# Project-MONAI/GenerativeModels

Measured on NVIDIA H100. Metric: ddim50_voxels_per_s, higher is better.
Workload: dtype fp16

## Files before the change

### generativemodels_b200/csrc/igemm.cu

```cuda
#include "common.cuh"
#include "wgmma.cuh"
#include <cuda.h>
#include <cudaTypedefs.h>
#include <mutex>
#include <string.h>

namespace b200 {

static constexpr int kBM = 128;
static constexpr int kBK = 64;
static constexpr int kABytes = kBM * kBK * 2;
static constexpr int kMmaWarp0 = 4;
static constexpr int kTmaWarp = 12;
static constexpr int kThreads = 13 * 32;

struct SegDev {
  int8_t src, dw, dh, dd;
  uint16_t c0, nchunks;
};

struct IgemmDev {
  alignas(64) CUtensorMap tmA[2];
  alignas(64) CUtensorMap tmB;
  const h16* a_ptr[2];
  int a_C[2], a_pitch[2];
  int in_N, in_D, in_H, in_W;
  int a_bcast;
  const h16* w_ptr;
  int w_rows, w_K, w_pitch;
  long long w_bstride;
  int w_batched;
  int n_seg, num_k_chunks;
  int sd, sh, sw;
  int N, OD, OH, OW;
  int BW, BH, BD, bw_log2, bh_log2;
  int tiles_w, tiles_h, tiles_d, tiles_n, num_tiles;
  int k_splits;
  long long split_stride;
  void* out_ptr;
  int out_dtype, cout, out_cols, out_vec, out_staged, out_v256;
  float* stat_ptr;
  float* gn_partial;
  int gn_slots, gn_slot0;
  int gn_sh;
  long long out_sN, out_sD, out_sH, out_sW;
  const float* bias;
  const float* rowvec;
  long long rowvec_bstride;
  const float* row_bias;
  int act1, act2;
  int geglu;
  float scale;
  const void* res_ptr;
  int res_dtype, res_vec, res_v256;
  long long res_sN, res_sD, res_sH, res_sW;
  SegDev seg[B200_IGEMM_MAX_SEG];
};

__device__ __forceinline__ void tma_load_5d(const CUtensorMap* tm, uint32_t bar, uint32_t dst, int c0,
                                            int c1, int c2, int c3, int c4) {
  asm volatile(
      "cp.async.bulk.tensor.5d.shared::cluster.global.mbarrier::complete_tx::bytes"
      " [%0], [%1, {%3, %4, %5, %6, %7}], [%2];" ::"r"(dst),
      "l"(reinterpret_cast<uint64_t>(tm)), "r"(bar), "r"(c0), "r"(c1), "r"(c2), "r"(c3), "r"(c4)
      : "memory");
}
template <int CH>
__device__ __forceinline__ void acc_ld(const float* src, uint32_t* r) {
#pragma unroll
  for (int j = 0; j < CH; j += 4) {
    const float4 t = *reinterpret_cast<const float4*>(src + j);
    r[j] = __float_as_uint(t.x); r[j + 1] = __float_as_uint(t.y);
    r[j + 2] = __float_as_uint(t.z); r[j + 3] = __float_as_uint(t.w);
  }
}

__host__ __device__ __forceinline__ int split_begin(int num_k, int splits, int ks) {
  return (int)(((long long)num_k * ks) / splits);
}

template <int CH>
__device__ __forceinline__ void epilogue_math(const IgemmDev& p, float* v, int nb, int ow, long long res_off,
                                              int col0) {
  const float rb = p.row_bias ? __ldg(p.row_bias + ow) : 0.f;
#pragma unroll
  for (int j = 0; j < CH; ++j) {
    int col = col0 + j;
    float add = rb;
    if (col < p.cout) {
      if (p.bias) add += __ldg(p.bias + col);
      if (p.rowvec) add += __ldg(p.rowvec + (long long)nb * p.rowvec_bstride + col);
    }
    float x = v[j] + add;
    x = apply_act(x, p.act1);
    v[j] = x * p.scale;
  }
  if (p.res_ptr) {
    if (p.res_dtype == B200_DT_H16) {
      const h16* r = reinterpret_cast<const h16*>(p.res_ptr) + res_off + col0;
      if (p.res_vec) {
#pragma unroll
        for (int g = 0; g < CH / 8; ++g) {
          if (col0 + g * 8 < p.out_cols) {
            uint4 t = __ldg(reinterpret_cast<const uint4*>(r + g * 8));
            float f[8];
            unpack8(t, f);
#pragma unroll
            for (int j = 0; j < 8; ++j) v[g * 8 + j] += f[j];
          }
        }
      } else {
#pragma unroll
        for (int j = 0; j < CH; ++j)
          if (col0 + j < p.out_cols) v[j] += h2f(r[j]);
      }
    } else {
      const float* r = reinterpret_cast<const float*>(p.res_ptr) + res_off + col0;
      if (p.res_vec) {
#pragma unroll
        for (int g = 0; g < CH / 4; ++g) {
          if (col0 + g * 4 < p.out_cols) {
            float4 t = __ldg(reinterpret_cast<const float4*>(r + g * 4));
            v[g * 4 + 0] += t.x; v[g * 4 + 1] += t.y; v[g * 4 + 2] += t.z; v[g * 4 + 3] += t.w;
          }
        }
      } else {
#pragma unroll
        for (int j = 0; j < CH; ++j)
          if (col0 + j < p.out_cols) v[j] += r[j];
      }
    }
  }
  if (p.act2 != B200_ACT_NONE) {
#pragma unroll
    for (int j = 0; j < CH; ++j) v[j] = apply_act(v[j], p.act2);
  }
#pragma unroll
  for (int j = 0; j < CH; ++j)
    if (col0 + j >= p.cout) v[j] = 0.f;
}

template <int CH>
__device__ __forceinline__ void store_direct(const IgemmDev& p, const float* v, long long out_off, int col0) {
  if (p.out_dtype == B200_DT_H16) {
    h16* o = reinterpret_cast<h16*>(p.out_ptr) + out_off + col0;
    if (p.out_vec) {
#pragma unroll
      for (int g = 0; g < CH / 8; ++g)
        if (col0 + g * 8 < p.out_cols) *reinterpret_cast<uint4*>(o + g * 8) = pack8(v + g * 8);
    } else {
#pragma unroll
      for (int j = 0; j < CH; ++j)
        if (col0 + j < p.out_cols) o[j] = f2h(v[j]);
    }
  } else {
    float* o = reinterpret_cast<float*>(p.out_ptr) + out_off + col0;
    if (p.out_vec) {
#pragma unroll
      for (int g = 0; g < CH / 4; ++g)
        if (col0 + g * 4 < p.out_cols)
          *reinterpret_cast<float4*>(o + g * 4) =
              make_float4(v[g * 4], v[g * 4 + 1], v[g * 4 + 2], v[g * 4 + 3]);
    } else {
#pragma unroll
      for (int j = 0; j < CH; ++j)
        if (col0 + j < p.out_cols) o[j] = v[j];
    }
  }
}


__device__ __forceinline__ void ldg256(const void* ptr, uint4& a, uint4& b) {
  a = __ldg(reinterpret_cast<const uint4*>(ptr));
  b = __ldg(reinterpret_cast<const uint4*>(ptr) + 1);
}
__device__ __forceinline__ void stg256(void* ptr, const uint4& a, const uint4& b) {
  reinterpret_cast<uint4*>(ptr)[0] = a;
  reinterpret_cast<uint4*>(ptr)[1] = b;
}
template <int CH>
__device__ __forceinline__ void act_inplace(float* v, int act) {
  if (act == B200_ACT_NONE) return;
  if (act == B200_ACT_SILU) {
#pragma unroll
    for (int j = 0; j < CH; ++j) v[j] = silu_f(v[j]);
  } else if (act == B200_ACT_LEAKYRELU || act == B200_ACT_LEAKYRELU02) {
    const float slope = act == B200_ACT_LEAKYRELU ? 0.01f : 0.2f;
#pragma unroll
    for (int j = 0; j < CH; ++j) v[j] = v[j] > 0.0f ? v[j] : slope * v[j];
  } else if (act == B200_ACT_GELU) {
#pragma unroll
    for (int j = 0; j < CH; ++j) v[j] = 0.5f * v[j] * (1.0f + erff(v[j] * 0.70710678118654752f));
  } else if (act == B200_ACT_TANH || act == B200_ACT_SIGMOID) {
#pragma unroll
    for (int j = 0; j < CH; ++j) v[j] = apply_act(v[j], act);
  } else {
#pragma unroll
    for (int j = 0; j < CH; ++j) v[j] = fmaxf(v[j], 0.0f);
  }
}
template <int CH>
__device__ __forceinline__ void load_res_fast(const IgemmDev& p, uint4* rv, long long res_off, int col0) {
  const h16* r = reinterpret_cast<const h16*>(p.res_ptr) + res_off + col0;
  if (p.res_v256) {
#pragma unroll
    for (int g = 0; g < CH / 16; ++g) ldg256(r + g * 16, rv[2 * g], rv[2 * g + 1]);
  } else {
#pragma unroll
    for (int g = 0; g < CH / 8; ++g) rv[g] = __ldg(reinterpret_cast<const uint4*>(r + g * 8));
  }
}
template <int CH>
__device__ __forceinline__ void epilogue_fast(const IgemmDev& p, const uint32_t* raw, const float* addv,
                                              const uint4* rv, long long out_off, int col0, float* gs) {
  float v[CH];
#pragma unroll
  for (int j = 0; j < CH; j += 4) {
    const float4 a = *reinterpret_cast<const float4*>(addv + j);
    v[j] = __uint_as_float(raw[j]) + a.x;
// ... 368 lines not shown
              h16* o = reinterpret_cast<h16*>(p.out_ptr) + out_off + ((n0 + c0) >> 1);
              uint4 pk[4];
#pragma unroll
              for (int g = 0; g < 4; ++g) pk[g] = pack8(v + g * 8);
              if (p.out_v256) {
                stg256(o, pk[0], pk[1]);
                stg256(o + 16, pk[2], pk[3]);
              } else {
#pragma unroll
                for (int g = 0; g < 4; ++g) *reinterpret_cast<uint4*>(o + g * 8) = pk[g];
              }
            }
          }
          c0 = BN;
        }
      }
      if (lean_ok) {
#pragma unroll 1
        for (; c0 < BN && n0 + c0 + CH <= p.cout; c0 += CH) {
          uint4 rv[CH / 8];
#pragma unroll
          for (int g = 0; g < CH / 8; ++g) rv[g] = rv_next[g];
          if (res_fast && c0 + CH < BN && n0 + c0 + 2 * CH <= p.cout)
            load_res_fast<CH>(p, rv_next, res_off, n0 + c0 + CH);
          uint32_t raw[CH];
          acc_ld<CH>(acc_row + c0, raw);
          if (row_ok) {
            if (p.res_ptr) epilogue_lean<CH, true>(p, raw, addv + c0, rv, out_off, n0 + c0);
            else epilogue_lean<CH, false>(p, raw, addv + c0, rv, out_off, n0 + c0);
          }
        }
      }
#pragma unroll 1
      for (; c0 < BN; c0 += CH) {
        if (n0 + c0 >= p.out_cols) break;
        if (fast_ok && n0 + c0 + CH <= p.cout) {
          uint4 rv[CH / 8];
#pragma unroll
          for (int g = 0; g < CH / 8; ++g) rv[g] = rv_next[g];
          if (res_fast && c0 + CH < BN && n0 + c0 + 2 * CH <= p.cout)
            load_res_fast<CH>(p, rv_next, res_off, n0 + c0 + CH);
          uint32_t raw[CH];
          acc_ld<CH>(acc_row + c0, raw);
          float gs[16] = {0.f, 0.f, 0.f, 0.f, 0.f, 0.f, 0.f, 0.f, 0.f, 0.f, 0.f, 0.f, 0.f, 0.f, 0.f, 0.f};
          if (row_ok) {
            if (p.row_bias) {
              const float rb = __ldg(p.row_bias + ow);
#pragma unroll
              for (int j = 0; j < CH; ++j) raw[j] = __float_as_uint(__uint_as_float(raw[j]) + rb);
            }
            epilogue_fast<CH>(p, raw, addv + c0, rv, out_off, n0 + c0, gn_on ? gs : nullptr);
          }
          if constexpr (CH == 32) {
            if (gn_on && p.gn_sh == 2) {
              float a8[8], a4[4], a2[2];
              bool hi = (lane & 16) != 0;
#pragma unroll
              for (int i = 0; i < 8; ++i) {
                const float send = hi ? gs[i] : gs[8 + i], keep = hi ? gs[8 + i] : gs[i];
                a8[i] = keep + __shfl_xor_sync(0xffffffffu, send, 16);
              }
              hi = (lane & 8) != 0;
#pragma unroll
              for (int i = 0; i < 4; ++i) {
                const float send = hi ? a8[i] : a8[4 + i], keep = hi ? a8[4 + i] : a8[i];
                a4[i] = keep + __shfl_xor_sync(0xffffffffu, send, 8);
              }
              hi = (lane & 4) != 0;
#pragma unroll
              for (int i = 0; i < 2; ++i) {
                const float send = hi ? a4[i] : a4[2 + i], keep = hi ? a4[2 + i] : a4[i];
                a2[i] = keep + __shfl_xor_sync(0xffffffffu, send, 4);
              }
              hi = (lane & 2) != 0;
              float c = (hi ? a2[1] : a2[0]) + __shfl_xor_sync(0xffffffffu, hi ? a2[0] : a2[1], 2);
              c += __shfl_xor_sync(0xffffffffu, c, 1);
              if ((lane & 1) == 0) {
                const int grp = (c0 >> 2) + ((lane >> 3) & 1) * 4 + ((lane >> 2) & 1) * 2 + ((lane >> 1) & 1);
                gacc[grp * 2 + (lane >> 4)] += c;
              }
            } else if (gn_on) {
              float a[4], b[2];
              bool hi = (lane & 16) != 0;
#pragma unroll
              for (int i = 0; i < 4; ++i) {
                const float send = hi ? gs[i] : gs[4 + i], keep = hi ? gs[4 + i] : gs[i];
                a[i] = keep + __shfl_xor_sync(0xffffffffu, send, 16);
              }
              hi = (lane & 8) != 0;
#pragma unroll
              for (int i = 0; i < 2; ++i) {
                const float send = hi ? a[i] : a[2 + i], keep = hi ? a[2 + i] : a[i];
                b[i] = keep + __shfl_xor_sync(0xffffffffu, send, 8);
              }
              hi = (lane & 4) != 0;
              float c = (hi ? b[1] : b[0]) + __shfl_xor_sync(0xffffffffu, hi ? b[0] : b[1], 4);
              c += __shfl_xor_sync(0xffffffffu, c, 2);
              c += __shfl_xor_sync(0xffffffffu, c, 1);
              if ((lane & 3) == 0) {
                const int grp = (c0 >> 3) + ((lane >> 3) & 1) * 2 + ((lane >> 2) & 1);
                gacc[grp * 2 + (lane >> 4)] += c;
              }
            }
          }
          continue;
        }
        uint32_t raw[CH];
        acc_ld<CH>(acc_row + c0, raw);
        float v[CH];
#pragma unroll
        for (int j = 0; j < CH; ++j) v[j] = __uint_as_float(raw[j]);
        if (row_ok) epilogue_math<CH>(p, v, nb, ow, res_off, n0 + c0);
        if (p.stat_ptr && row_ok) {
          float cmax = -INFINITY;
#pragma unroll
          for (int j = 0; j < CH; ++j)
            if (n0 + c0 + j < p.cout) cmax = fmaxf(cmax, v[j]);
          if (cmax > -INFINITY) {
            const float nm = fmaxf(run_max, cmax);
            float acc = 0.f;
#pragma unroll
            for (int j = 0; j < CH; ++j)
              if (n0 + c0 + j < p.cout) acc += __expf(v[j] - nm);
            run_sum = run_sum * __expf(run_max - nm) + acc;
            run_max = nm;
          }
        }
        if (p.out_staged) store_staged<CH>(p, v, my_tile, row_ok, out_off, n0 + c0, lane);
        else if (row_ok) store_direct<CH>(p, v, out_off, n0 + c0);
      }
      if (p.stat_ptr && row_ok) {
        float2* st = reinterpret_cast<float2*>(p.stat_ptr) + ((long long)ow * p.tiles_n + nt);
        *st = make_float2(run_max, run_sum);
      }
      if (want_key >= 0) {
#pragma unroll
        for (int i = 0; i < PER; ++i)
          if (lane + 32 * i < BN) addv_other[lane + 32 * i] = nbv[i] + nrw[i];
        next_key = want_key;
      }
      __syncwarp();
      if (lane == 0) mbar_arrive(tempty_bar);
    }
    if (gn_on) { __syncwarp(); gn_flush(); }
  }

  __syncthreads();
}

namespace wide {
static constexpr int kThreads = 384;
static constexpr int kCluster = 2;
static constexpr int kBN = 256;
static constexpr int kStages = 4;
static constexpr int kBHalfBytes = 128 * kBK * 2;
static constexpr int kStageBytes = kABytes + 2 * kBHalfBytes;
static constexpr int kSliceLd = 36;
static constexpr int kOffSlice = kStages * kStageBytes;
static constexpr int kOffAdd = kOffSlice + 8 * 16 * kSliceLd * 4;
static constexpr int kOffBar = kOffAdd + 8 * kBN * 4;
static constexpr int kSmem = 1024 + kOffBar + 2 * kStages * 8;
static constexpr int kProducerRegs = 40, kConsumerRegs = 232;
static_assert(kProducerRegs * 128 + kConsumerRegs * 256 <= 65536, "register budget of one CTA per SM");
}

__device__ __forceinline__ float gn_reduce16(const float* gs, int lane, int gn_sh) {
  const bool h3 = (lane & 8) != 0, h2 = (lane & 4) != 0, h1 = (lane & 2) != 0;
  if (gn_sh == 3) {
    float a[2];
#pragma unroll
    for (int i = 0; i < 2; ++i) a[i] = (h3 ? gs[2 + i] : gs[i]) + __shfl_xor_sync(0xffffffffu, h3 ? gs[i] : gs[2 + i], 8);
    float c = (h2 ? a[1] : a[0]) + __shfl_xor_sync(0xffffffffu, h2 ? a[0] : a[1], 4);
    c += __shfl_xor_sync(0xffffffffu, c, 2);
    c += __shfl_xor_sync(0xffffffffu, c, 1);
    return c;
  }
  float a4[4], a2[2];
#pragma unroll
  for (int i = 0; i < 4; ++i) a4[i] = (h3 ? gs[4 + i] : gs[i]) + __shfl_xor_sync(0xffffffffu, h3 ? gs[i] : gs[4 + i], 8);
#pragma unroll
  for (int i = 0; i < 2; ++i) a2[i] = (h2 ? a4[2 + i] : a4[i]) + __shfl_xor_sync(0xffffffffu, h2 ? a4[i] : a4[2 + i], 4);
  float c = (h1 ? a2[1] : a2[0]) + __shfl_xor_sync(0xffffffffu, h1 ? a2[0] : a2[1], 2);
  c += __shfl_xor_sync(0xffffffffu, c, 1);
  return c;
}

__global__ void __launch_bounds__(wide::kThreads, 1) igemm_wide_kernel(const __grid_constant__ IgemmDev p) {
  using namespace wide;
  extern __shared__ uint8_t smem_raw[];
  uint8_t* sm = smem_raw + ((1024u - (smem_u32(smem_raw) & 1023u)) & 1023u);
  const uint32_t ring = smem_u32(sm);
  const uint32_t full0 = ring + kOffBar, empty0 = full0 + 8 * kStages;

  const int tid = threadIdx.x;
  const int wg = __shfl_sync(0xffffffffu, tid >> 7, 0);
  const uint32_t rank = cluster_ctarank();
  const int cid = (int)blockIdx.x / kCluster, n_clusters = (int)gridDim.x / kCluster;
  const int m_tiles = p.tiles_w * p.tiles_h * p.tiles_d * p.N;
  const int num_units = p.num_tiles;
  const int num_k = p.num_k_chunks;

  if (tid == 0) {
    for (int s = 0; s < kStages; ++s) {
      mbar_init(full0 + 8 * s, 1);
      mbar_init(empty0 + 8 * s, 8 * kCluster);
    }
    asm volatile("fence.mbarrier_init.release.cluster;" ::: "memory");
  }
  cluster_sync();

  struct MTile { int nt, wt, ht, dt, nb; bool ok; };
  auto unit_tile = [&](int u) {
    MTile t;
    t.nt = u % p.tiles_n;
    int m = 2 * (u / p.tiles_n) + (int)rank;
    t.ok = m < m_tiles;
    if (!t.ok) m = m_tiles - 1;
    t.wt = m % p.tiles_w; m /= p.tiles_w;
    t.ht = m % p.tiles_h; m /= p.tiles_h;
    t.dt = m % p.tiles_d;
    t.nb = m / p.tiles_d;
    return t;
  };

  if (wg == 0) {
    setmaxnreg_dec<kProducerRegs>();
    if (tid == 0) {
      int stage = 0;
      uint32_t phase = 0;
      for (int u = cid; u < num_units; u += n_clusters) {
        const MTile t = unit_tile(u);
        const int iw0 = t.wt * p.BW * p.sw, ih0 = t.ht * p.BH * p.sh, id0 = t.dt * p.BD * p.sd;
        const int wrow = t.nt * kBN + 128 * (int)rank;
        int kglob = 0;
        for (int s = 0; s < p.n_seg; ++s) {
          const SegDev sg = p.seg[s];
          const CUtensorMap* tm = &p.tmA[sg.src];
          const int cw = iw0 + sg.dw, ch = ih0 + sg.dh, cd = id0 + sg.dd;
          for (int c = 0; c < sg.nchunks; ++c, ++kglob) {
            mbar_wait(empty0 + 8 * stage, phase ^ 1u);
            const uint32_t dst = ring + stage * kStageBytes, fb = full0 + 8 * stage;
            mbar_arrive_expect_tx(fb, kStageBytes);
            tma_load_5d(tm, fb, dst, (sg.c0 + c) * kBK, cw, ch, cd, t.nb);
            tma_load_3d_multicast(&p.tmB, fb, dst + kABytes + rank * kBHalfBytes, kglob * kBK, wrow, 0, 0x3);
            if (++stage == kStages) { stage = 0; phase ^= 1u; }
          }
        }
      }
    }
  } else {
    setmaxnreg_inc<kConsumerRegs>();
    const int c = wg - 1;
    const int wq = (tid >> 5) & 3;
    const int lane = tid & 31;
    float* slice = reinterpret_cast<float*>(sm + kOffSlice) + (4 * c + wq) * 16 * kSliceLd;
    float* addv = reinterpret_cast<float*>(sm + kOffAdd) + (4 * c + wq) * kBN;
    const int er = 64 * c + 16 * wq + (lane & 15);
    const int eh = lane >> 4;
    const int rw = er & (p.BW - 1), rh = (er >> p.bw_log2) & (p.BH - 1), rd = er >> (p.bw_log2 + p.bh_log2);
    auto release = [&](int s) {
      __syncwarp();
      if (lane == 0) {
        mbar_arrive_cluster(empty0 + 8 * s, 0);
        mbar_arrive_cluster(empty0 + 8 * s, 1);
      }
    };

    const bool gn_on = p.gn_partial != nullptr;
    const int gsh = p.gn_sh;
    float gacc[kBN / 32];
#pragma unroll
    for (int s = 0; s < kBN / 32; ++s) gacc[s] = 0.f;
    int key = -1, gn_nb = 0, gn_n0 = 0;
    auto gn_flush = [&]() {
      const bool writer = (lane & (gsh == 3 ? 3 : 1)) == 0;
      const int stat = (lane >> 3) & 1;
      const int gl = gsh == 3 ? (lane >> 2) & 1 : ((lane >> 1) & 3);
      float* dst = p.gn_partial +
                   (((long long)gn_nb * p.gn_slots + p.gn_slot0 + 4 * blockIdx.x + wq) * (p.cout >> gsh)) * 2 + stat;
      for (int pass = 0; pass < 2; ++pass) {
        if (pass == c && writer) {
#pragma unroll
          for (int s = 0; s < kBN / 32; ++s) dst[(((gn_n0 + 32 * s + 16 * eh) >> gsh) + gl) * 2] += gacc[s];
        }
        if (pass == 0) named_sync(1, 256);
      }
#pragma unroll
      for (int s = 0; s < kBN / 32; ++s) gacc[s] = 0.f;
    };

    float acc[kBN / 2];
    int stage = 0;
    uint32_t phase = 0;
    for (int u = cid; u < num_units; u += n_clusters) {
      int prev = -1;
      for (int k = 0; k < num_k; ++k) {
        mbar_wait(full0 + 8 * stage, phase);
        const uint32_t st = ring + stage * kStageBytes;
        const uint64_t adesc = wgmma_desc(st + c * (64 * kBK * 2));
        const uint64_t bdesc = wgmma_desc(st + kABytes);
        wgmma_fence();
#pragma unroll
        for (int kk = 0; kk < kBK / 16; ++kk)
          wgmma_ss<kBN>(acc, adesc + 2u * kk, bdesc + 2u * kk, (k | kk) != 0 ? 1u : 0u);
        wgmma_commit();
        wgmma_wait<1>();
        if (prev >= 0) release(prev);
        prev = stage;
        if (++stage == kStages) { stage = 0; phase ^= 1u; }
      }
      wgmma_wait<0>();
      wgmma_touch<kBN / 2>(acc);
      release(prev);

      const MTile t = unit_tile(u);
      const int n0 = t.nt * kBN;
      const int ow = t.wt * p.BW + rw, oh = t.ht * p.BH + rh, od = t.dt * p.BD + rd;
      const bool row_ok = t.ok && ow < p.OW && oh < p.OH && od < p.OD;
      const long long out_off = t.nb * p.out_sN + od * p.out_sD + oh * p.out_sH + ow * p.out_sW;
      const long long res_off = t.nb * p.res_sN + od * p.res_sD + oh * p.res_sH + ow * p.res_sW;
      if (t.nb * p.tiles_n + t.nt != key) {
        if (gn_on && key >= 0) gn_flush();
        key = t.nb * p.tiles_n + t.nt;
        gn_nb = t.nb;
        gn_n0 = n0;
        float bv[kBN / 32], rv[kBN / 32];
#pragma unroll
        for (int i = 0; i < kBN / 32; ++i) {
          const int col = n0 + lane + 32 * i;
          bv[i] = p.bias ? __ldg(p.bias + col) : 0.f;
          rv[i] = p.rowvec ? __ldg(p.rowvec + (long long)t.nb * p.rowvec_bstride + col) : 0.f;
        }
        __syncwarp();
#pragma unroll
        for (int i = 0; i < kBN / 32; ++i) addv[lane + 32 * i] = bv[i] + rv[i];
        __syncwarp();
      }
      const bool res_on = p.res_ptr && row_ok;
      uint4 rv_next[2] = {make_uint4(0u, 0u, 0u, 0u), make_uint4(0u, 0u, 0u, 0u)};
      if (res_on) load_res_fast<16>(p, rv_next, res_off, n0 + 16 * eh);
#pragma unroll
      for (int s = 0; s < kBN / 32; ++s) {
        __syncwarp();
#pragma unroll
        for (int j = 4 * s; j < 4 * s + 4; ++j) {
          const int col = 8 * (j - 4 * s) + 2 * (lane & 3);
          *reinterpret_cast<float2*>(slice + (lane >> 2) * kSliceLd + col) = make_float2(acc[4 * j], acc[4 * j + 1]);
          *reinterpret_cast<float2*>(slice + ((lane >> 2) + 8) * kSliceLd + col) =
              make_float2(acc[4 * j + 2], acc[4 * j + 3]);
        }
        __syncwarp();
        uint32_t raw[16];
        acc_ld<16>(slice + (lane & 15) * kSliceLd + 16 * eh, raw);
        const uint4 rv[2] = {rv_next[0], rv_next[1]};
        if (res_on && s + 1 < kBN / 32) load_res_fast<16>(p, rv_next, res_off, n0 + 32 * (s + 1) + 16 * eh);
        const int cc = 32 * s + 16 * eh;
        float gs[8] = {0.f, 0.f, 0.f, 0.f, 0.f, 0.f, 0.f, 0.f};
        if (row_ok) epilogue_fast<16>(p, raw, addv + cc, rv, out_off, n0 + cc, gs);
        if (gn_on) gacc[s] += gn_reduce16(gs, lane, gsh);
      }
    }
    if (gn_on && key >= 0) gn_flush();
  }
  cluster_sync();
}

__global__ void igemm_check_kernel(const __grid_constant__ IgemmDev p) {
  const long long rows = (long long)p.N * p.OD * p.OH * p.OW;
  const int col_groups = (p.out_cols + 15) / 16;
  const long long idx = (long long)blockIdx.x * blockDim.x + threadIdx.x;
  if (idx >= rows * col_groups) return;
  const int cg = (int)(idx % col_groups);
  long long m = idx / col_groups;
  const int ow = (int)(m % p.OW); m /= p.OW;
  const int oh = (int)(m % p.OH); m /= p.OH;
  const int od = (int)(m % p.OD); m /= p.OD;
  const int nb = (int)m;
  float acc[16];
#pragma unroll
  for (int j = 0; j < 16; ++j) acc[j] = 0.f;
  const int wb = p.w_batched ? nb : 0;
  const h16* wbase = p.w_ptr + (long long)wb * p.w_bstride;
  int kglob = 0;
  for (int s = 0; s < p.n_seg; ++s) {
    const SegDev sg = p.seg[s];
    const int iw = ow * p.sw + sg.dw, ih = oh * p.sh + sg.dh, id = od * p.sd + sg.dd;
    const bool inb = iw >= 0 && iw < p.in_W && ih >= 0 && ih < p.in_H && id >= 0 && id < p.in_D;
    const h16* a = p.a_ptr[sg.src] +
        ((((long long)(p.a_bcast ? 0 : nb) * p.in_D + id) * p.in_H + ih) * p.in_W + iw) * p.a_pitch[sg.src];
    for (int c = 0; c < sg.nchunks; ++c, ++kglob) {
      if (!inb) continue;
      for (int e = 0; e < kBK; ++e) {
        const int ch = (sg.c0 + c) * kBK + e;
        const int kk = kglob * kBK + e;
        if (ch >= p.a_C[sg.src] || kk >= p.w_K) break;
        const float av = h2f(a[ch]);
#pragma unroll
        for (int j = 0; j < 16; ++j) {
          const int col = cg * 16 + j;
          if (col < p.w_rows) acc[j] += av * h2f(wbase[(long long)col * p.w_pitch + kk]);
        }
      }
    }
  }
  const long long out_off = nb * p.out_sN + od * p.out_sD + oh * p.out_sH + ow * p.out_sW;
  const long long res_off = nb * p.res_sN + od * p.res_sD + oh * p.res_sH + ow * p.res_sW;
  epilogue_row<16>(p, acc, nb, ow, out_off, res_off, cg * 16);
}

static PFN_cuTensorMapEncodeTiled g_encode = nullptr;
static std::once_flag g_encode_once;

static void load_encode() {
  void* fn = nullptr;
  cudaDriverEntryPointQueryResult qres;
  if (cudaGetDriverEntryPoint("cuTensorMapEncodeTiled", &fn, cudaEnableDefault, &qres) == cudaSuccess &&
      qres == cudaDriverEntryPointSuccess)
    g_encode = reinterpret_cast<PFN_cuTensorMapEncodeTiled>(fn);
}

static int ilog2(int v) {
  int l = 0;
  while ((1 << l) < v) ++l;
  return l;
}

struct TileShape { int bw, bh, bd; };

static TileShape choose_tile(int OW, int OH, int OD, int sw, int sh, int sd) {
  static const TileShape cands[] = {{128, 1, 1}, {64, 2, 1}, {32, 4, 1}, {16, 8, 1}, {8, 16, 1},
                                    {4, 32, 1},  {32, 2, 2}, {16, 4, 2}, {8, 8, 2},  {16, 2, 4},
                                    {8, 4, 4},   {4, 8, 4},  {4, 4, 8},  {8, 2, 8},  {2, 8, 8},
                                    {4, 2, 16},  {2, 4, 16}, {2, 2, 32}, {1, 1, 128}, {1, 128, 1},
                                    {2, 64, 1},  {1, 8, 16}, {1, 16, 8}};
  double best = 1e30;
  TileShape bt = cands[0];
  for (const TileShape& c : cands) {
    if (c.bw * sw > 256 || c.bh * sh > 256 || c.bd * sd > 256) continue;
    double tw = (double)((OW + c.bw - 1) / c.bw) * c.bw;
    double th = (double)((OH + c.bh - 1) / c.bh) * c.bh;
    double td = (double)((OD + c.bd - 1) / c.bd) * c.bd;
    double cost = tw * th * td;
    cost *= (1.0 + 1e-3 * (7 - ilog2(c.bw)));
    if (cost < best) { best = cost; bt = c; }
  }
  return bt;
}

__global__ void gn8_partial_check_kernel(const __grid_constant__ IgemmDev p) {
  const long long rows = (long long)p.N * p.OD * p.OH * p.OW;
  const int gw = 1 << p.gn_sh;
  const int groups = p.cout >> p.gn_sh;
  const long long idx = (long long)blockIdx.x * blockDim.x + threadIdx.x;
  if (idx >= rows * groups) return;
  const int g = (int)(idx % groups);
  long long m = idx / groups;
  const int ow = (int)(m % p.OW); m /= p.OW;
  const int oh = (int)(m % p.OH); m /= p.OH;
  const int od = (int)(m % p.OD); m /= p.OD;
  const int nb = (int)m;
  const h16* o = reinterpret_cast<const h16*>(p.out_ptr) + nb * p.out_sN + od * p.out_sD +
                           oh * p.out_sH + ow * p.out_sW + g * gw;
  float s = 0.f, q = 0.f;
  for (int j = 0; j < gw; ++j) { const float f = h2f(o[j]); s += f; q = fmaf(f, f, q); }
  float* dst = p.gn_partial + (((long long)nb * p.gn_slots + p.gn_slot0) * groups + g) * 2;
  atomicAdd(dst, s);
  atomicAdd(dst + 1, q);
}

__global__ void __launch_bounds__(256) igemm_split_reduce_kernel(const IgemmDev p, const float* __restrict__ ws,
                                                                 int splits, int ws_cols, long long ws_stride) {
  const int groups = (p.out_cols + 7) >> 3;
  const long long rows = (long long)p.N * p.OD * p.OH * p.OW;
  const long long idx = blockIdx.x * (long long)blockDim.x + threadIdx.x;
  if (idx >= rows * groups) return;
  const int col0 = (int)(idx % groups) * 8;
  const long long row = idx / groups;
  long long t = row;
  const int ow = (int)(t % p.OW); t /= p.OW;
  const int oh = (int)(t % p.OH); t /= p.OH;
  const int od = (int)(t % p.OD); t /= p.OD;
  const int nb = (int)t;
  float v[8] = {0.f, 0.f, 0.f, 0.f, 0.f, 0.f, 0.f, 0.f};
  const float* src = ws + row * ws_cols + col0;
  int s = 0;
  for (; s + 8 <= splits; s += 8, src += 8 * ws_stride) {
    float4 a[8], b[8];
#pragma unroll
    for (int j = 0; j < 8; ++j) {
      a[j] = __ldg(reinterpret_cast<const float4*>(src + j * ws_stride));
      b[j] = __ldg(reinterpret_cast<const float4*>(src + j * ws_stride + 4));
    }
#pragma unroll
    for (int j = 0; j < 8; ++j) {
      v[0] += a[j].x; v[1] += a[j].y; v[2] += a[j].z; v[3] += a[j].w;
      v[4] += b[j].x; v[5] += b[j].y; v[6] += b[j].z; v[7] += b[j].w;
    }
  }
  if (s + 4 <= splits) {
    float4 a[4], b[4];
#pragma unroll
    for (int j = 0; j < 4; ++j) {
      a[j] = __ldg(reinterpret_cast<const float4*>(src + j * ws_stride));
      b[j] = __ldg(reinterpret_cast<const float4*>(src + j * ws_stride + 4));
    }
#pragma unroll
    for (int j = 0; j < 4; ++j) {
      v[0] += a[j].x; v[1] += a[j].y; v[2] += a[j].z; v[3] += a[j].w;
      v[4] += b[j].x; v[5] += b[j].y; v[6] += b[j].z; v[7] += b[j].w;
    }
    s += 4; src += 4 * ws_stride;
  }
  if (s + 2 <= splits) {
    const float4 a0 = __ldg(reinterpret_cast<const float4*>(src)), b0 = __ldg(reinterpret_cast<const float4*>(src + 4));
    const float4 a1 = __ldg(reinterpret_cast<const float4*>(src + ws_stride));
// ... 367 lines not shown
```

Measured before the change: 145,500.

## Stage wide-kernel epilogue through shared memory with bulk residual loads and row stores

```diff
diff --git a/generativemodels_b200/csrc/igemm.cu b/generativemodels_b200/csrc/igemm.cu
--- a/generativemodels_b200/csrc/igemm.cu
+++ b/generativemodels_b200/csrc/igemm.cu
@@ -65,6 +65,14 @@
       "l"(reinterpret_cast<uint64_t>(tm)), "r"(bar), "r"(c0), "r"(c1), "r"(c2), "r"(c3), "r"(c4)
       : "memory");
 }
+__device__ __forceinline__ void bulk_load(uint32_t dst, const void* src, uint32_t bytes, uint32_t bar) {
+  asm volatile("cp.async.bulk.shared::cluster.global.mbarrier::complete_tx::bytes [%0], [%1], %2, [%3];"
+               ::"r"(dst), "l"(src), "r"(bytes), "r"(bar) : "memory");
+}
+__device__ __forceinline__ void bulk_store(void* dst, uint32_t src, uint32_t bytes) {
+  asm volatile("cp.async.bulk.global.shared::cta.bulk_group [%0], [%1], %2;" ::"l"(dst), "r"(src), "r"(bytes)
+               : "memory");
+}
 template <int CH>
 __device__ __forceinline__ void acc_ld(const float* src, uint32_t* r) {
 #pragma unroll
@@ -739,35 +747,30 @@
 static constexpr int kThreads = 384;
 static constexpr int kCluster = 2;
 static constexpr int kBN = 256;
-static constexpr int kStages = 4;
+static constexpr int kStages = 3;
 static constexpr int kBHalfBytes = 128 * kBK * 2;
 static constexpr int kStageBytes = kABytes + 2 * kBHalfBytes;
-static constexpr int kSliceLd = 36;
-static constexpr int kOffSlice = kStages * kStageBytes;
-static constexpr int kOffAdd = kOffSlice + 8 * 16 * kSliceLd * 4;
+static constexpr int kRowBytes = kBN * 2;
+static constexpr int kStgLd = kRowBytes + 16;
+static constexpr int kOffStg = kStages * kStageBytes;
+static constexpr int kOffAdd = kOffStg + kBM * kStgLd;
 static constexpr int kOffBar = kOffAdd + 8 * kBN * 4;
-static constexpr int kSmem = 1024 + kOffBar + 2 * kStages * 8;
+static constexpr int kSmem = 1024 + kOffBar + (2 * kStages + 2) * 8;
 static constexpr int kProducerRegs = 40, kConsumerRegs = 232;
 static_assert(kProducerRegs * 128 + kConsumerRegs * 256 <= 65536, "register budget of one CTA per SM");
 }
 
-__device__ __forceinline__ float gn_reduce16(const float* gs, int lane, int gn_sh) {
-  const bool h3 = (lane & 8) != 0, h2 = (lane & 4) != 0, h1 = (lane & 2) != 0;
-  if (gn_sh == 3) {
-    float a[2];
-#pragma unroll
-    for (int i = 0; i < 2; ++i) a[i] = (h3 ? gs[2 + i] : gs[i]) + __shfl_xor_sync(0xffffffffu, h3 ? gs[i] : gs[2 + i], 8);
-    float c = (h2 ? a[1] : a[0]) + __shfl_xor_sync(0xffffffffu, h2 ? a[0] : a[1], 4);
-    c += __shfl_xor_sync(0xffffffffu, c, 2);
-    c += __shfl_xor_sync(0xffffffffu, c, 1);
-    return c;
-  }
-  float a4[4], a2[2];
-#pragma unroll
-  for (int i = 0; i < 4; ++i) a4[i] = (h3 ? gs[4 + i] : gs[i]) + __shfl_xor_sync(0xffffffffu, h3 ? gs[i] : gs[4 + i], 8);
-#pragma unroll
-  for (int i = 0; i < 2; ++i) a2[i] = (h2 ? a4[2 + i] : a4[i]) + __shfl_xor_sync(0xffffffffu, h2 ? a4[i] : a4[2 + i], 4);
-  float c = (h1 ? a2[1] : a2[0]) + __shfl_xor_sync(0xffffffffu, h1 ? a2[0] : a2[1], 2);
+__device__ __forceinline__ float gn_reduce_slice(const float* s, int lane, int gn_sh) {
+  float a[4], b[2];
+  bool hi = (lane & 16) != 0;
+#pragma unroll
+  for (int i = 0; i < 4; ++i) a[i] = (hi ? s[4 + i] : s[i]) + __shfl_xor_sync(0xffffffffu, hi ? s[i] : s[4 + i], 16);
+  hi = (lane & 8) != 0;
+#pragma unroll
+  for (int i = 0; i < 2; ++i) b[i] = (hi ? a[2 + i] : a[i]) + __shfl_xor_sync(0xffffffffu, hi ? a[i] : a[2 + i], 8);
+  hi = (lane & 4) != 0;
+  float c = (hi ? b[1] : b[0]) + __shfl_xor_sync(0xffffffffu, hi ? b[0] : b[1], 4);
+  if (gn_sh == 3) c += __shfl_xor_sync(0xffffffffu, c, 2);
   c += __shfl_xor_sync(0xffffffffu, c, 1);
   return c;
 }
@@ -778,6 +781,7 @@
   uint8_t* sm = smem_raw + ((1024u - (smem_u32(smem_raw) & 1023u)) & 1023u);
   const uint32_t ring = smem_u32(sm);
   const uint32_t full0 = ring + kOffBar, empty0 = full0 + 8 * kStages;
+  const uint32_t stg = ring + kOffStg, stg_full = empty0 + 8 * kStages, stg_empty = stg_full + 8;
 
   const int tid = threadIdx.x;
   const int wg = __shfl_sync(0xffffffffu, tid >> 7, 0);
@@ -792,6 +796,8 @@
       mbar_init(full0 + 8 * s, 1);
       mbar_init(empty0 + 8 * s, 8 * kCluster);
     }
+    mbar_init(stg_full, 1);
+    mbar_init(stg_empty, 8);
     asm volatile("fence.mbarrier_init.release.cluster;" ::: "memory");
   }
   cluster_sync();
@@ -809,9 +815,16 @@
     t.nb = m / p.tiles_d;
     return t;
   };
+  auto tile_row = [&](const MTile& t, int r, int& ow, int& oh, int& od) {
+    ow = t.wt * p.BW + (r & (p.BW - 1));
+    oh = t.ht * p.BH + ((r >> p.bw_log2) & (p.BH - 1));
+    od = t.dt * p.BD + (r >> (p.bw_log2 + p.bh_log2));
+    return t.ok && ow < p.OW && oh < p.OH && od < p.OD;
+  };
 
   if (wg == 0) {
     setmaxnreg_dec<kProducerRegs>();
+    const int warp = __shfl_sync(0xffffffffu, tid >> 5, 0);
     if (tid == 0) {
       int stage = 0;
       uint32_t phase = 0;
@@ -834,17 +847,36 @@
           }
         }
       }
+    } else if (warp == 1 && p.res_ptr) {
+      const int lane = tid & 31;
+      uint32_t it = 0;
+      for (int u = cid; u < num_units; u += n_clusters, ++it) {
+        const MTile t = unit_tile(u);
+        mbar_wait(stg_empty, (it & 1u) ^ 1u);
+        int ow, oh, od, rows = 0;
+#pragma unroll
+        for (int i = 0; i < kBM / 32; ++i) rows += __popc(__ballot_sync(0xffffffffu, tile_row(t, lane + 32 * i, ow, oh, od)));
+        if (lane == 0) mbar_arrive_expect_tx(stg_full, rows * kRowBytes);
+        __syncwarp();
+#pragma unroll
+        for (int i = 0; i < kBM / 32; ++i) {
+          const int r = lane + 32 * i;
+          if (tile_row(t, r, ow, oh, od)) {
+            const h16* src = reinterpret_cast<const h16*>(p.res_ptr) + t.nb * p.res_sN + od * p.res_sD +
+                             oh * p.res_sH + ow * p.res_sW + t.nt * kBN;
+            bulk_load(stg + r * kStgLd, src, kRowBytes, stg_full);
+          }
+        }
+      }
     }
   } else {
     setmaxnreg_inc<kConsumerRegs>();
     const int c = wg - 1;
     const int wq = (tid >> 5) & 3;
     const int lane = tid & 31;
-    float* slice = reinterpret_cast<float*>(sm + kOffSlice) + (4 * c + wq) * 16 * kSliceLd;
     float* addv = reinterpret_cast<float*>(sm + kOffAdd) + (4 * c + wq) * kBN;
-    const int er = 64 * c + 16 * wq + (lane & 15);
-    const int eh = lane >> 4;
-    const int rw = er & (p.BW - 1), rh = (er >> p.bw_log2) & (p.BH - 1), rd = er >> (p.bw_log2 + p.bh_log2);
+    const int r0 = 64 * c + 16 * wq + (lane >> 2);
+    uint8_t* stg_r0 = sm + kOffStg + r0 * kStgLd + 4 * (lane & 3);
     auto release = [&](int s) {
       __syncwarp();
       if (lane == 0) {
@@ -861,14 +893,14 @@
     int key = -1, gn_nb = 0, gn_n0 = 0;
     auto gn_flush = [&]() {
       const bool writer = (lane & (gsh == 3 ? 3 : 1)) == 0;
-      const int stat = (lane >> 3) & 1;
-      const int gl = gsh == 3 ? (lane >> 2) & 1 : ((lane >> 1) & 3);
+      const int stat = lane >> 4;
+      const int gc = 8 * ((lane >> 2) & 3) + (gsh == 3 ? 0 : 4 * ((lane >> 1) & 1));
       float* dst = p.gn_partial +
                    (((long long)gn_nb * p.gn_slots + p.gn_slot0 + 4 * blockIdx.x + wq) * (p.cout >> gsh)) * 2 + stat;
       for (int pass = 0; pass < 2; ++pass) {
         if (pass == c && writer) {
 #pragma unroll
-          for (int s = 0; s < kBN / 32; ++s) dst[(((gn_n0 + 32 * s + 16 * eh) >> gsh) + gl) * 2] += gacc[s];
+          for (int s = 0; s < kBN / 32; ++s) dst[((gn_n0 + 32 * s + gc) >> gsh) * 2] += gacc[s];
         }
         if (pass == 0) named_sync(1, 256);
       }
@@ -878,8 +910,8 @@
 
     float acc[kBN / 2];
     int stage = 0;
-    uint32_t phase = 0;
-    for (int u = cid; u < num_units; u += n_clusters) {
+    uint32_t phase = 0, it = 0;
+    for (int u = cid; u < num_units; u += n_clusters, ++it) {
       int prev = -1;
       for (int k = 0; k < num_k; ++k) {
         mbar_wait(full0 + 8 * stage, phase);
@@ -902,10 +934,8 @@
 
       const MTile t = unit_tile(u);
       const int n0 = t.nt * kBN;
-      const int ow = t.wt * p.BW + rw, oh = t.ht * p.BH + rh, od = t.dt * p.BD + rd;
-      const bool row_ok = t.ok && ow < p.OW && oh < p.OH && od < p.OD;
-      const long long out_off = t.nb * p.out_sN + od * p.out_sD + oh * p.out_sH + ow * p.out_sW;
-      const long long res_off = t.nb * p.res_sN + od * p.res_sD + oh * p.res_sH + ow * p.res_sW;
+      int ow, oh, od;
+      const bool ok0 = tile_row(t, r0, ow, oh, od), ok8 = tile_row(t, r0 + 8, ow, oh, od);
       if (t.nb * p.tiles_n + t.nt != key) {
         if (gn_on && key >= 0) gn_flush();
         key = t.nb * p.tiles_n + t.nt;
@@ -923,31 +953,64 @@
         for (int i = 0; i < kBN / 32; ++i) addv[lane + 32 * i] = bv[i] + rv[i];
         __syncwarp();
       }
-      const bool res_on = p.res_ptr && row_ok;
-      uint4 rv_next[2] = {make_uint4(0u, 0u, 0u, 0u), make_uint4(0u, 0u, 0u, 0u)};
-      if (res_on) load_res_fast<16>(p, rv_next, res_off, n0 + 16 * eh);
+      if (p.res_ptr) mbar_wait(stg_full, it & 1u);
 #pragma unroll
       for (int s = 0; s < kBN / 32; ++s) {
-        __syncwarp();
-#pragma unroll
-        for (int j = 4 * s; j < 4 * s + 4; ++j) {
-          const int col = 8 * (j - 4 * s) + 2 * (lane & 3);
-          *reinterpret_cast<float2*>(slice + (lane >> 2) * kSliceLd + col) = make_float2(acc[4 * j], acc[4 * j + 1]);
-          *reinterpret_cast<float2*>(slice + ((lane >> 2) + 8) * kSliceLd + col) =
-              make_float2(acc[4 * j + 2], acc[4 * j + 3]);
-        }
-        __syncwarp();
-        uint32_t raw[16];
-        acc_ld<16>(slice + (lane & 15) * kSliceLd + 16 * eh, raw);
-        const uint4 rv[2] = {rv_next[0], rv_next[1]};
-        if (res_on && s + 1 < kBN / 32) load_res_fast<16>(p, rv_next, res_off, n0 + 32 * (s + 1) + 16 * eh);
-        const int cc = 32 * s + 16 * eh;
-        float gs[8] = {0.f, 0.f, 0.f, 0.f, 0.f, 0.f, 0.f, 0.f};
-        if (row_ok) epilogue_fast<16>(p, raw, addv + cc, rv, out_off, n0 + cc, gs);
-        if (gn_on) gacc[s] += gn_reduce16(gs, lane, gsh);
-      }
+        float v[16];
+#pragma unroll
+        for (int i = 0; i < 4; ++i) {
+          const int j = 4 * s + i;
+          const float2 a = *reinterpret_cast<const float2*>(addv + 8 * j + 2 * (lane & 3));
+          v[4 * i] = acc[4 * j] + a.x;
+          v[4 * i + 1] = acc[4 * j + 1] + a.y;
+          v[4 * i + 2] = acc[4 * j + 2] + a.x;
+          v[4 * i + 3] = acc[4 * j + 3] + a.y;
+        }
+        act_inplace<16>(v, p.act1);
+        if (p.scale != 1.0f) {
+#pragma unroll
+          for (int j = 0; j < 16; ++j) v[j] *= p.scale;
+        }
+        if (p.res_ptr) {
+#pragma unroll
+          for (int i = 0; i < 4; ++i) {
+            const float2 f0 = h22f2(*reinterpret_cast<const h162*>(stg_r0 + 16 * (4 * s + i)));
+            const float2 f8 = h22f2(*reinterpret_cast<const h162*>(stg_r0 + 8 * kStgLd + 16 * (4 * s + i)));
+            v[4 * i] += f0.x; v[4 * i + 1] += f0.y; v[4 * i + 2] += f8.x; v[4 * i + 3] += f8.y;
+          }
+        }
+        act_inplace<16>(v, p.act2);
+        float gs[8];
+#pragma unroll
+        for (int i = 0; i < 4; ++i) {
+          const h162 h0 = f2h2(v[4 * i], v[4 * i + 1]), h8 = f2h2(v[4 * i + 2], v[4 * i + 3]);
+          *reinterpret_cast<h162*>(stg_r0 + 16 * (4 * s + i)) = h0;
+          *reinterpret_cast<h162*>(stg_r0 + 8 * kStgLd + 16 * (4 * s + i)) = h8;
+          float2 f0 = h22f2(h0), f8 = h22f2(h8);
+          if (!ok0) f0 = make_float2(0.f, 0.f);
+          if (!ok8) f8 = make_float2(0.f, 0.f);
+          gs[i] = (f0.x + f0.y) + (f8.x + f8.y);
+          gs[4 + i] = fmaf(f8.y, f8.y, fmaf(f8.x, f8.x, fmaf(f0.y, f0.y, f0.x * f0.x)));
+        }
+        if (gn_on) gacc[s] += gn_reduce_slice(gs, lane, gsh);
+      }
+      asm volatile("fence.proxy.async.shared::cta;" ::: "memory");
+      __syncwarp();
+      if (lane < 16) {
+        const int r = 64 * c + 16 * wq + lane;
+        if (tile_row(t, r, ow, oh, od)) {
+          h16* dst = reinterpret_cast<h16*>(p.out_ptr) + t.nb * p.out_sN + od * p.out_sD + oh * p.out_sH +
+                     ow * p.out_sW + n0;
+          bulk_store(dst, stg + r * kStgLd, kRowBytes);
+        }
+        asm volatile("cp.async.bulk.commit_group;" ::: "memory");
+        asm volatile("cp.async.bulk.wait_group.read 0;" ::: "memory");
+      }
+      __syncwarp();
+      if (lane == 0) mbar_arrive(stg_empty);
     }
     if (gn_on && key >= 0) gn_flush();
+    asm volatile("cp.async.bulk.wait_group 0;" ::: "memory");
   }
   cluster_sync();
 }
```

Result: faster. 147,200, median of 6 (+1.2%).
